# Hiroto1201/Open3D-ML

Measured on AMD Instinct MI355X. Metric: Mpoints/s neighbor-search + sparse-conv fwd; RandLA-Net frames/s, higher is better.
Workload: dtype f32; 1 GPU; C1 fixed_radius_search: layers.FixedRadiusSearch forward (hash build + search) over 64 scenes/GPU x 65,536 U[0,1)^3 pts, r=0.05, L2, int32 idx; scenes_per_gpu=64, parallelism=scene-dp1

## Files before the change

### open3d-ml_amd/csrc/nns_frs.hip

```cpp
#include <algorithm>
#include <cstdlib>
#include <mutex>

#include "primitives.hpp"
#include "spatial_hash.hpp"

namespace o3dml {

__global__ void __launch_bounds__(256) gather_sorted_points_kernel(const float* __restrict__ points,
                                                                   const uint32_t* __restrict__ index, int64_t n,
                                                                   float4* __restrict__ out, int sentinel,
                                                                   int64_t* __restrict__ zero_a, int n_zero_a,
                                                                   int64_t* __restrict__ zero_b) {
    const int64_t per = ceil_div(n, static_cast<int64_t>(gridDim.x));
    const int64_t blk = xcd_block();
    const int64_t e = min(n, (blk + 1) * per);
    constexpr int U = 4;
    for (int64_t j0 = blk * per + threadIdx.x; j0 < e; j0 += U * static_cast<int64_t>(blockDim.x)) {
        uint32_t id[U];
#pragma unroll
        for (int u = 0; u < U; ++u) {
            const int64_t j = j0 + u * static_cast<int64_t>(blockDim.x);
            id[u] = j < e ? index[j] : 0u;
        }
        float x[U], y[U], z[U];
#pragma unroll
        for (int u = 0; u < U; ++u) {
            x[u] = points[3 * static_cast<int64_t>(id[u])];
            y[u] = points[3 * static_cast<int64_t>(id[u]) + 1];
            z[u] = points[3 * static_cast<int64_t>(id[u]) + 2];
        }
#pragma unroll
        for (int u = 0; u < U; ++u) {
            const int64_t j = j0 + u * static_cast<int64_t>(blockDim.x);
            if (j < e) out[j] = make_float4(x[u], y[u], z[u], __uint_as_float(id[u]));
        }
    }
    if (blockIdx.x == 0 && threadIdx.x == 0) {
        if (sentinel) {
            const float inf = __builtin_huge_valf();
            out[n] = make_float4(inf, inf, inf, 0.f);
        }
        for (int j = 0; j < n_zero_a; ++j) zero_a[j] = 0;
        if (zero_b) *zero_b = 0;
    }
}

#ifndef O3DML_FRS_ROWCAP
#define O3DML_FRS_ROWCAP 64
#endif
constexpr int kRowCap = O3DML_FRS_ROWCAP;
static_assert(kRowCap >= 1 && kRowCap <= 64, "the row copy takes one row per wave instruction");
constexpr int kDirWords = 24;

struct LaneSplitTab {
    uint32_t v[65];
    constexpr LaneSplitTab() : v() {
        for (int ng = 0; ng <= 64; ++ng) {
            const uint32_t S = ng == 0 ? 64u : 64u / static_cast<uint32_t>(ng);
            v[ng] = S | (((65536u + S - 1u) / S) << 8);
        }
    }
};
__constant__ constexpr LaneSplitTab kLaneSplitTab{};
#define kLaneSplit kLaneSplitTab.v

#ifndef O3DML_DIAG
#define O3DML_DIAG 0
#endif
#ifndef O3DML_STREAM_U
#define O3DML_STREAM_U 2
#endif
#ifndef O3DML_FRS_DMA
#define O3DML_FRS_DMA 0
#endif
typedef __attribute__((address_space(3))) void* frs_lds_ptr;
#ifndef O3DML_FRS_OOBST
#define O3DML_FRS_OOBST 0
#endif
constexpr int kStreamU = O3DML_STREAM_U;
constexpr int kCandCap = 256;

#ifndef O3DML_FRS_DPPMIN
#define O3DML_FRS_DPPMIN 1
#endif
template <int CTRL>
__device__ __forceinline__ float dpp_f(float v) {
    return __int_as_float(__builtin_amdgcn_update_dpp(0, __float_as_int(v), CTRL, 0xF, 0xF, false));
}
#define O3DML_DPP_STEP(NAME, OP, CTRL)                                                                   \
    __device__ __forceinline__ float NAME(float v) {                                                    \
        float r;                                                                                        \
        asm volatile("s_nop 1\n\t" OP "_dpp %0, %1, %1 " CTRL " row_mask:0xf bank_mask:0xf"            \
                     : "=v"(r)                                                                          \
                     : "v"(v));                                                                         \
        return r;                                                                                       \
    }
O3DML_DPP_STEP(dmin_q1, "v_min_f32", "quad_perm:[1,0,3,2]")
O3DML_DPP_STEP(dmin_q2, "v_min_f32", "quad_perm:[2,3,0,1]")
O3DML_DPP_STEP(dmin_hm, "v_min_f32", "row_half_mirror")
O3DML_DPP_STEP(dmin_rm, "v_min_f32", "row_mirror")
O3DML_DPP_STEP(dmax_q1, "v_max_f32", "quad_perm:[1,0,3,2]")
O3DML_DPP_STEP(dmax_q2, "v_max_f32", "quad_perm:[2,3,0,1]")
O3DML_DPP_STEP(dmax_hm, "v_max_f32", "row_half_mirror")
O3DML_DPP_STEP(dmax_rm, "v_max_f32", "row_mirror")
#undef O3DML_DPP_STEP
template <bool MAX>
__device__ __forceinline__ float row_ext_f(float v) {
#if O3DML_FRS_DPPMIN
    if constexpr (MAX) return dmax_rm(dmax_hm(dmax_q2(dmax_q1(v))));
    return dmin_rm(dmin_hm(dmin_q2(dmin_q1(v))));
#else
    auto op = [](float a, float b) { return MAX ? fmaxf(a, b) : fminf(a, b); };
    v = op(v, dpp_f<0xB1>(v));
    v = op(v, dpp_f<0x4E>(v));
    v = op(v, dpp_f<0x141>(v));
    v = op(v, dpp_f<0x140>(v));
    return v;
#endif
}
__device__ __forceinline__ float rdlane_f(float v, int l) {
    return __int_as_float(__builtin_amdgcn_readlane(__float_as_int(v), l));
}
__device__ __forceinline__ float wave_min_f(float v) {
    v = row_ext_f<false>(v);
    return fminf(fminf(rdlane_f(v, 0), rdlane_f(v, 16)), fminf(rdlane_f(v, 32), rdlane_f(v, 48)));
}
__device__ __forceinline__ float wave_max_f(float v) {
    v = row_ext_f<true>(v);
    return fmaxf(fmaxf(rdlane_f(v, 0), rdlane_f(v, 16)), fmaxf(rdlane_f(v, 32), rdlane_f(v, 48)));
}
__device__ __forceinline__ float row0_min_f(float v) { return rdlane_f(row_ext_f<false>(v), 0); }
__device__ __forceinline__ float row0_max_f(float v) { return rdlane_f(row_ext_f<true>(v), 0); }

template <int METRIC>
__device__ __forceinline__ float box_dist(const float4& p, float lx, float ly, float lz, float hx, float hy,
                                          float hz) {
    const float gx = p.x - __builtin_amdgcn_fmed3f(p.x, lx, hx);
    const float gy = p.y - __builtin_amdgcn_fmed3f(p.y, ly, hy);
    const float gz = p.z - __builtin_amdgcn_fmed3f(p.z, lz, hz);
    if constexpr (METRIC == kL2) {
        return __builtin_fmaf(gz, gz, __builtin_fmaf(gy, gy, gx * gx));
    } else if constexpr (METRIC == kL1) {
        return (fabsf(gx) + fabsf(gy)) + fabsf(gz);
    } else {
        const float ax = fabsf(gx), ay = fabsf(gy), az = fabsf(gz);
        const float m = ax > ay ? ax : ay;
        return m > az ? m : az;
    }
}

template <int METRIC>
__device__ __forceinline__ float box_box_dist(float alx, float aly, float alz, float ahx, float ahy, float ahz,
                                              float blx, float bly, float blz, float bhx, float bhy, float bhz) {
    const float gx = fmaxf(fmaxf(alx - bhx, blx - ahx), 0.f);
    const float gy = fmaxf(fmaxf(aly - bhy, bly - ahy), 0.f);
    const float gz = fmaxf(fmaxf(alz - bhz, blz - ahz), 0.f);
    if constexpr (METRIC == kL2) {
        return __builtin_fmaf(gz, gz, __builtin_fmaf(gy, gy, gx * gx));
    } else if constexpr (METRIC == kL1) {
        return (gx + gy) + gz;
    } else {
        const float m = gx > gy ? gx : gy;
        return m > gz ? m : gz;
    }
}

__device__ __forceinline__ int keep_slot(uint64_t km) {
    return static_cast<int>(__builtin_amdgcn_mbcnt_hi(static_cast<uint32_t>(km >> 32),
                                                      __builtin_amdgcn_mbcnt_lo(static_cast<uint32_t>(km), 0u)));
}

__device__ __forceinline__ uint32_t mbcnt64(uint64_t m) {
    return __builtin_amdgcn_mbcnt_hi(static_cast<uint32_t>(m >> 32),
                                     __builtin_amdgcn_mbcnt_lo(static_cast<uint32_t>(m), 0u));
}

__device__ __forceinline__ uint32_t bcnt_add(uint32_t x, uint32_t acc) {
    uint32_t r;
    asm("v_bcnt_u32_b32 %0, %1, %2" : "=v"(r) : "v"(x), "v"(acc));
    return r;
}

__device__ __forceinline__ uint32_t rdlane(int v, uint32_t lane) {
    return static_cast<uint32_t>(__builtin_amdgcn_readlane(v, static_cast<int>(lane)));
}

__device__ __forceinline__ int32_t float_key(float f) {
    const int32_t i = __float_as_int(f);
    return i ^ ((i >> 31) & 0x7fffffff);
}
__device__ __forceinline__ uint32_t key_float(int32_t k) {
    return static_cast<uint32_t>(k ^ ((k >> 31) & 0x7fffffff));
}

#ifndef O3DML_FRS_NUM_SGPR
#define O3DML_FRS_NUM_SGPR 80
#endif
#ifndef O3DML_FRS_WAVES
#define O3DML_FRS_WAVES 8
#endif
#ifndef O3DML_FRS_ABS16
#define O3DML_FRS_ABS16 1
#endif
#define O3DML_FRS_ATTR \
    __attribute__((amdgpu_num_sgpr(O3DML_FRS_NUM_SGPR), amdgpu_waves_per_eu(DIST ? 1 : O3DML_FRS_WAVES, 8)))
template <int METRIC, bool IGNORE, bool DIST, int MODE, class TIdx, bool REL16>
__global__ void __launch_bounds__(64) O3DML_FRS_ATTR
frs_group_kernel(const float4* __restrict__ pts, uint32_t n_pts, const uint32_t* __restrict__ cs,
                 const float4* __restrict__ qpts, const uint32_t* __restrict__ qsel,
                 const uint32_t* __restrict__ qkeys, int bshift, int64_t m_host, const int64_t* __restrict__ m_dev,
                 float r, float inv, float thr, int nb, const int64_t* __restrict__ qrs,
                 const uint32_t* __restrict__ hts, const int64_t* __restrict__ prs,
                 uint32_t* __restrict__ counts, uint32_t* __restrict__ tidx,
                 float* __restrict__ tdist, uint32_t* __restrict__ over, int64_t* __restrict__ n_over,
                 const int64_t* __restrict__ rs, TIdx* __restrict__ out_idx, float* __restrict__ out_dist,
                 const int64_t* __restrict__ total, int64_t cap, const uint32_t* __restrict__ dir,
                 int64_t dir_cap, int qlog, int64_t dense_w) {
    __shared__ float4 cand[kCandCap];
    __shared__ float4 qsh[64];
    __shared__ int64_t qrow[MODE == 0 ? 1 : 64];
    const int lane = threadIdx.x;
    const float inf = __builtin_huge_valf();
    const float4 far = make_float4(inf, inf, inf, 0.f);
    const int64_t m = MODE == 1 && cap >= 0 && *total > cap ? 0 : (m_dev ? *m_dev : m_host);
    const int64_t nchunks = MODE == 0 ? (m + (1 << qlog) - 1) >> qlog : m;
    const bool pts_rsrc_ok = n_pts < 0x07FFFFFEu;
    const bool sub = dir != nullptr && static_cast<int64_t>(hts[nb]) <= dir_cap;
    const __amdgpu_buffer_rsrc_t rows_rsrc = __builtin_amdgcn_make_buffer_rsrc(
            tidx, static_cast<short>(0), REL16 ? static_cast<int>(m * 2 * kRowCap) : 0, kBufferFlags);
    const __amdgpu_buffer_rsrc_t pts_rsrc = __builtin_amdgcn_make_buffer_rsrc(
            const_cast<float4*>(pts), static_cast<short>(0), static_cast<int>((2u * n_pts + 1u) * 16u), kBufferFlags);
    const int64_t per = (nchunks + 7) >> 3;
    const bool xcd_map = static_cast<int64_t>(gridDim.x) == 8 * per;
    int64_t chunk = xcd_map ? static_cast<int64_t>(blockIdx.x & 7) * per + (blockIdx.x >> 3) : blockIdx.x;
    for (; chunk < nchunks; chunk = xcd_map ? nchunks : chunk + gridDim.x) {
        const int64_t t = MODE == 0 ? (chunk << qlog) + lane : chunk;
        const bool valid = t < m && (MODE == 0 ? lane < (1 << qlog) : lane == 0);
        float4 q4 = far;
        QueryBins qb;
#pragma unroll
        for (int k = 0; k < 9; ++k) qb.b[k] = 0xffffffffu;
        int64_t row = 0;
        uint32_t pbase = 0;
        if (valid) {
            if constexpr (MODE == 0) {
                if (qsel) {
                    const uint32_t qs = qsel[t];
                    if (qpts) {
                        const float* qp = reinterpret_cast<const float*>(qpts) + 3 * static_cast<int64_t>(qs);
                        q4 = make_float4(qp[0], qp[1], qp[2], __uint_as_float(qs));
                    } else {
                        q4 = pts[qs];
                    }
                } else {
                    q4 = qpts[t];
                }
            } else {
                const uint32_t id = over[t];
                const float* qp = reinterpret_cast<const float*>(qpts) + 3 * static_cast<int64_t>(id);
                q4 = make_float4(qp[0], qp[1], qp[2], __uint_as_float(id));
            }
            const uint32_t qid = __float_as_uint(q4.w);
            const int b = qkeys ? (bshift >= 32 ? 0 : static_cast<int>(qkeys[t] >> bshift)) : batch_of(qid, qrs, nb);
            if constexpr (REL16) pbase = static_cast<uint32_t>(prs[b]);
            const uint32_t first = hts[b], tsize = hts[b + 1] - first;
            qb = query_bins(q4.x, q4.y, q4.z, r, inv, first, tsize);
            if constexpr (MODE == 1) row = dense_w > 0 ? static_cast<int64_t>(qid) * dense_w : rs[qid];
        }
        uint64_t todo = __builtin_amdgcn_ballot_w64(valid);
        int ngrp = 0;
        uint32_t goff = 0;
        uint32_t mytag = 0;
        int vgrp = 0;
        while (todo) {
            const int leader = __builtin_ctzll(todo);
            bool same = valid;
#pragma unroll
            for (int k = 0; k < 9; ++k) same = same && qb.b[k] == rdlane(static_cast<int>(qb.b[k]), leader);
            const uint64_t gm = __builtin_amdgcn_ballot_w64(same);
            todo &= ~gm;
            const uint32_t ng = static_cast<uint32_t>(__popcll(gm));
            if (same) {
                const uint32_t slot = mbcnt64(gm);
                mytag = static_cast<uint32_t>(ngrp) | (slot == 0 ? 0x300u : 0x200u) | ((goff + slot) << 16);
            }
            if (lane == ngrp) vgrp = static_cast<int>(ng | (goff << 8) | (static_cast<uint32_t>(leader) << 16));
            goff += ng;
            ++ngrp;
        }
        uint32_t* const tab = reinterpret_cast<uint32_t*>(cand);
        __syncthreads();
        if (valid) {
            qsh[mytag >> 16] = q4;
            if constexpr (MODE == 1) qrow[mytag >> 16] = row;
        }
        uint32_t vst = 0, vlen = 0;
        uint64_t km = 0;
        int gi = 0, nbat = 0;
        for (int grp = 0; grp < ngrp; ++grp, ++gi) {
            if (gi == nbat) {
                uint2* const seg = reinterpret_cast<uint2*>(cand) + 64;
                int bl = lane;
                uint32_t kmax = INT32_MAX, kmin = static_cast<uint32_t>(INT32_MIN), zero = 0u;
                asm volatile("" : "+v"(bl), "+v"(kmax), "+v"(kmin), "+v"(zero));
                const int tg = (bl * 57) >> 9, tk = bl - 9 * tg;
                __syncthreads();
                const uint32_t rel = (mytag & 0xffu) - static_cast<uint32_t>(grp);
                if ((mytag & 0x100u) != 0u && rel < 7u) {
                    uint4* const tp = reinterpret_cast<uint4*>(tab) + 4 * rel;
                    tp[0] = make_uint4(kmax, kmax, kmax, kmin);
                    tp[1] = make_uint4(kmin, kmin, qb.b[0], qb.b[1]);
                    tp[2] = make_uint4(qb.b[2], qb.b[3], qb.b[4], qb.b[5]);
                    tp[3] = make_uint4(qb.b[6], qb.b[7], qb.b[8], zero);
                }
                seg[bl] = make_uint2(zero, zero);
                __syncthreads();
                if ((mytag & 0x200u) != 0u && rel < 7u) {
                    const float4 me = qsh[mytag >> 16];
                    int32_t* const k = reinterpret_cast<int32_t*>(tab) + 16 * rel;
                    const int32_t kx = float_key(me.x), ky = float_key(me.y), kz = float_key(me.z);
                    __hip_atomic_fetch_min(k + 0, kx, __ATOMIC_RELAXED, __HIP_MEMORY_SCOPE_WORKGROUP);
                    __hip_atomic_fetch_min(k + 1, ky, __ATOMIC_RELAXED, __HIP_MEMORY_SCOPE_WORKGROUP);
                    __hip_atomic_fetch_min(k + 2, kz, __ATOMIC_RELAXED, __HIP_MEMORY_SCOPE_WORKGROUP);
                    __hip_atomic_fetch_max(k + 3, kx, __ATOMIC_RELAXED, __HIP_MEMORY_SCOPE_WORKGROUP);
                    __hip_atomic_fetch_max(k + 4, ky, __ATOMIC_RELAXED, __HIP_MEMORY_SCOPE_WORKGROUP);
                    __hip_atomic_fetch_max(k + 5, kz, __ATOMIC_RELAXED, __HIP_MEMORY_SCOPE_WORKGROUP);
                }
                __syncthreads();
                const bool task_ok = tg < 7 && grp + tg < ngrp;
                const uint32_t* const tq = tab + 16 * tg;
                const uint32_t vb = tab[task_ok ? 16 * tg + 6 + tk : 6];
                const uint32_t prev = tq[5 + tk];
                const uint4 b0 = reinterpret_cast<const uint4*>(tq)[0];
                const uint2 b1 = reinterpret_cast<const uint2*>(tq)[2];
                const uint32_t s0 = cs[vb], e0 = cs[vb + 1];
                uint4 w0 = {}, w1 = {}, w2 = {}, w3 = {}, w4 = {}, w5 = {};
                if (sub) {
                    const uint4* dp = reinterpret_cast<const uint4*>(dir + static_cast<size_t>(vb) * kDirWords);
                    w0 = dp[0], w1 = dp[1], w2 = dp[2], w3 = dp[3], w4 = dp[4], w5 = dp[5];
                }
                const bool first = task_ok && e0 > s0 && (tk == 0 || prev != vb);
                uint32_t st = s0, ln = e0 - s0;
                if (first && sub) {
                    auto f = [](uint32_t u) { return __uint_as_float(u); };
                    auto kf = [](uint32_t k) { return __uint_as_float(key_float(static_cast<int32_t>(k))); };
                    const float lx = kf(b0.x), ly = kf(b0.y), lz = kf(b0.z), hx = kf(b0.w), hy = kf(b1.x),
                                hz = kf(b1.y);
                    const uint32_t n0 = w0.x, n1 = w0.y, n2 = ln - n0 - n1;
                    const bool r0 = n0 > 0 && box_box_dist<METRIC>(f(w1.x), f(w1.y), f(w1.z), f(w1.w), f(w2.x),
                                                                   f(w2.y), lx, ly, lz, hx, hy, hz) <= thr;
                    const bool r1 = n1 > 0 && box_box_dist<METRIC>(f(w2.z), f(w2.w), f(w3.x), f(w3.y), f(w3.z),
                                                                   f(w3.w), lx, ly, lz, hx, hy, hz) <= thr;
                    const bool r2 = n2 > 0 && box_box_dist<METRIC>(f(w4.x), f(w4.y), f(w4.z), f(w4.w), f(w5.x),
                                                                   f(w5.y), lx, ly, lz, hx, hy, hz) <= thr;
                    const int nr = static_cast<int>(r0) + static_cast<int>(r1) + static_cast<int>(r2);
                    const uint32_t base = n_pts + 1 + s0;
                    if (nr == 0) {
                        ln = 0;
                    } else if (nr == 1) {
                        st = r0 && n0 == ln ? s0 : base + (r0 ? 0u : (r1 ? n0 : n0 + n1));
                        ln = r0 ? n0 : (r1 ? n1 : n2);
                    }
                }
                const bool live = first && ln > 0;
                km = __builtin_amdgcn_ballot_w64(live);
                nbat = __popcll(km) > 57 ? 6 : min(7, ngrp - grp);
                if (live && tg < nbat) seg[mbcnt64(km) + tg] = make_uint2(st, ln);
                __syncthreads();
                const uint2 sg = seg[bl];
                vst = sg.x, vlen = sg.y;
                __syncthreads();
                gi = 0;
            }
            const uint32_t ginfo = rdlane(vgrp, static_cast<uint32_t>(grp));
            const int ng = static_cast<int>(ginfo & 0xffu);
            const uint32_t gslot = (ginfo >> 8) & 0xffu, leader = ginfo >> 16;
            const uint32_t gbase = REL16 ? rdlane(static_cast<int>(pbase), leader) : 0u;
            float lx, ly, lz, hx, hy, hz;
            if (ng <= 16) {
                const float4 v = lane < ng ? qsh[gslot + (lane & 15)] : far;
                const float4 w = lane < ng ? v : make_float4(-inf, -inf, -inf, 0.f);
                lx = row0_min_f(v.x), ly = row0_min_f(v.y), lz = row0_min_f(v.z);
                hx = row0_max_f(w.x), hy = row0_max_f(w.y), hz = row0_max_f(w.z);
            } else {
                const float4 v = lane < ng ? qsh[gslot + lane] : far;
                const float4 w = lane < ng ? v : make_float4(-inf, -inf, -inf, 0.f);
                lx = wave_min_f(v.x), ly = wave_min_f(v.y), lz = wave_min_f(v.z);
                hx = wave_max_f(w.x), hy = wave_max_f(w.y), hz = wave_max_f(w.z);
            }
            const uint32_t split = kLaneSplit[ng];
            const int S = static_cast<int>(split & 0xffu);
            const int g = static_cast<int>((static_cast<uint32_t>(lane) * (split >> 8)) >> 16);
            const int sl = lane - g * S;
            float4 mq = far;
            int64_t mrow = 0;
            if (g < ng) {
                mq = qsh[gslot + g];
                mrow = MODE == 0 ? static_cast<int64_t>(__float_as_uint(mq.w)) : qrow[gslot + g];
            }
            uint32_t cnt = 0;
            const uint32_t row_b = static_cast<uint32_t>(mrow) * (2u * kRowCap);
            const uint64_t gmask = S == 64 ? ~0ull : (g < ng ? ((1ull << S) - 1ull) << (g * S) : 0ull);
            const uint32_t gm_lo = static_cast<uint32_t>(gmask), gm_hi = static_cast<uint32_t>(gmask >> 32);
            int bk = __popcll(km & ((1ull << (9 * gi)) - 1ull)) + gi;
            int nbk = bk + __popcll((km >> (9 * gi)) & 0x1ffull);
#if O3DML_DIAG == 2
            nbk = bk;
#endif
            const int fill_lim = kCandCap - 64 * kStreamU - (S - 1);
            uint32_t boff = 0;
            auto round_src = [&]() -> uint32_t {
                if (bk >= nbk) return n_pts;
                const uint32_t st0 = rdlane(static_cast<int>(vst), bk) + boff;
                const uint32_t t = rdlane(static_cast<int>(vlen), bk) - boff;
                if (t > 64) {
                    boff += 64;
                    return st0 + lane;
                }
                const uint32_t n1 = rdlane(static_cast<int>(vlen), bk + 1);
                const uint32_t d1 = rdlane(static_cast<int>(vst), bk + 1) - t;
                const uint32_t src = static_cast<uint32_t>(lane) < t ? st0 + lane : d1 + lane;
                if (t + n1 <= 64) {
                    bk += 2;
                    boff = 0;
                } else {
                    bk += 1;
                    boff = 64 - t;
                }
                return static_cast<uint32_t>(lane) < t + n1 ? src : n_pts;
            };
            auto load_step = [&](float4* c, auto buf) {
                uint32_t src[kStreamU];
#pragma unroll
                for (int u = 0; u < kStreamU; ++u) src[u] = round_src();
                if constexpr (decltype(buf)::value) {
#pragma unroll
                    for (int u = 0; u < kStreamU; ++u)
                        c[u] = __builtin_bit_cast(float4,
                                                  __builtin_amdgcn_raw_buffer_load_b128(pts_rsrc, src[u] * 16u, 0, 0));
                } else {
#pragma unroll
                    for (int u = 0; u < kStreamU; ++u) c[u] = pts[src[u]];
                }
            };
            auto stream_and_test = [&](auto buf) {
            int nc = 0;
            while (true) {
#if O3DML_FRS_DMA
                if constexpr (decltype(buf)::value) {
                    while (bk < nbk && nc <= fill_lim) {
                        uint32_t src[kStreamU];
#pragma unroll
                        for (int u = 0; u < kStreamU; ++u) src[u] = round_src();
                        const int nc0 = nc;
#pragma unroll
                        for (int u = 0; u < kStreamU; ++u)
                            __builtin_amdgcn_raw_ptr_buffer_load_lds(pts_rsrc, (frs_lds_ptr)(cand + nc0 + 64 * u), 16,
                                                                     src[u] * 16u, 0, 0, 0);
                        asm volatile("s_waitcnt vmcnt(0)" ::: "memory");
#pragma unroll
                        for (int u = 0; u < kStreamU; ++u) {
                            float4 c = cand[nc0 + 64 * u + lane];
                            const bool keep = box_dist<METRIC>(c, lx, ly, lz, hx, hy, hz) <= thr;
                            const uint64_t km = __builtin_amdgcn_ballot_w64(keep);
                            if constexpr (REL16 && !O3DML_FRS_ABS16) c.w = __uint_as_float(__float_as_uint(c.w) - gbase);
                            if (keep)
                                (cand + nc)[keep_slot(km)] = c;
                            nc += __popcll(km);
                        }
                    }
                }
                while (!decltype(buf)::value && bk < nbk && nc <= fill_lim) {
#else
                while (bk < nbk && nc <= fill_lim) {
#endif
                    float4 c[kStreamU];
                    load_step(c, buf);
#pragma unroll
                    for (int u = 0; u < kStreamU; ++u) {
                        const bool keep = box_dist<METRIC>(c[u], lx, ly, lz, hx, hy, hz) <= thr;
                        const uint64_t km = __builtin_amdgcn_ballot_w64(keep);
                        if constexpr (REL16 && !O3DML_FRS_ABS16)
                            c[u].w = __uint_as_float(__float_as_uint(c[u].w) - gbase);
                        if (keep)
                            (cand + nc)[keep_slot(km)] = c[u];
                        nc += __popcll(km);
                    }
                }
                const int ncp = static_cast<int>(((static_cast<uint32_t>(nc + S - 1) * (split >> 8)) >> 16) *
                                                 static_cast<uint32_t>(S));
                if (nc + lane < ncp) cand[nc + lane] = far;
                __syncthreads();
#if O3DML_DIAG == 0
                auto test = [&](float4 p) {
                    asm volatile("" : "+v"(p.w));
                    const float d = dist_metric<METRIC>(p.x, p.y, p.z, mq.x, mq.y, mq.z);
                    const bool hit = d <= thr && !(IGNORE && p.x == mq.x && p.y == mq.y && p.z == mq.z);
                    const uint64_t bal = __builtin_amdgcn_ballot_w64(hit);
                    const uint32_t mlo = static_cast<uint32_t>(bal) & gm_lo;
                    const uint32_t mhi = static_cast<uint32_t>(bal >> 32) & gm_hi;
#if O3DML_FRS_OOBST
                    if constexpr (MODE == 0 && REL16 && !DIST) {
                        const uint32_t pos = __builtin_amdgcn_mbcnt_hi(mhi, __builtin_amdgcn_mbcnt_lo(mlo, cnt));
                        const uint32_t ps = min(pos, static_cast<uint32_t>(kRowCap - 1));
                        __builtin_amdgcn_raw_buffer_store_b16(static_cast<unsigned short>(__float_as_uint(p.w)),
                                                              rows_rsrc, hit ? row_b + (ps << 1) : 0x80000000u, 0,
                                                              0);
                        cnt = bcnt_add(mhi, bcnt_add(mlo, cnt));
                        return;
                    }
#endif
                    if (hit) {
                        const uint32_t pos = __builtin_amdgcn_mbcnt_hi(mhi, __builtin_amdgcn_mbcnt_lo(mlo, cnt));
                        if constexpr (MODE == 0) {
                            const uint32_t ps = min(pos, static_cast<uint32_t>(kRowCap - 1));
                            if constexpr (REL16)
                                __builtin_amdgcn_raw_buffer_store_b16(
                                        static_cast<unsigned short>(__float_as_uint(p.w)), rows_rsrc,
                                        row_b + (ps << 1), 0, 0);
                            else
                                tidx[mrow * kRowCap + ps] = __float_as_uint(p.w);
                            if constexpr (DIST) tdist[mrow * kRowCap + ps] = d;
                        } else {
                            out_idx[mrow + pos] = static_cast<TIdx>(__float_as_uint(p.w));
                            if constexpr (DIST) out_dist[mrow + pos] = d;
                        }
                    }
                    cnt = bcnt_add(mhi, bcnt_add(mlo, cnt));
                };
                int e0 = 0;
                for (; e0 + 4 * S <= ncp; e0 += 4 * S) {
                    float4 p[4];
#pragma unroll
                    for (int u = 0; u < 4; ++u) p[u] = cand[e0 + u * S + sl];
#pragma unroll
                    for (int u = 0; u < 4; ++u) test(p[u]);
                }
                for (; e0 < ncp; e0 += S) test(cand[e0 + sl]);
#endif
                __syncthreads();
                nc = 0;
                if (bk >= nbk) break;
            }
            };
            if (pts_rsrc_ok)
                stream_and_test(std::true_type{});
            else
                stream_and_test(std::false_type{});
            if constexpr (MODE == 0) {
                if (g < ng && sl == 0) {
                    counts[__float_as_uint(mq.w)] = cnt;
                    if (cnt > static_cast<uint32_t>(kRowCap))
                        over[atomicAdd(reinterpret_cast<unsigned long long*>(n_over), 1ull)] =
                                static_cast<uint32_t>(mrow);
                }
            }
        }
    }
}

__device__ uint32_t g_frs_zero[4];
#ifndef O3DML_COPY_ROWS
#define O3DML_COPY_ROWS 64
#endif
constexpr int kCopyRows = O3DML_COPY_ROWS;

template <bool DIST, bool REL16, class TIdx>
__global__ void __launch_bounds__(256) group_rows_copy_kernel(int64_t m, const uint32_t* __restrict__ counts,
                                                              const int64_t* __restrict__ rs,
                                                              const int64_t* __restrict__ qrs,
                                                              const int64_t* __restrict__ prs, int nb,
                                                              const uint32_t* __restrict__ tidx,
                                                              const float* __restrict__ tdist,
                                                              TIdx* __restrict__ idx, float* __restrict__ dist,
                                                              int64_t cap) {
    if (cap >= 0 && rs[m] > cap) return;
    const int lane = threadIdx.x & 63;
    const int64_t wave = (static_cast<int64_t>(blockIdx.x) * blockDim.x + threadIdx.x) >> 6;
    const int64_t nwaves = (static_cast<int64_t>(gridDim.x) * blockDim.x) >> 6;
    const uint16_t* t16 = reinterpret_cast<const uint16_t*>(tidx);
    for (int64_t base = wave * 64; base < m; base += nwaves * 64) {
        const int64_t t = base + lane;
        int n = 0;
        int64_t o = 0;
        uint32_t pb = 0;
        if constexpr (REL16) {
            const int64_t ub = static_cast<int64_t>(__builtin_amdgcn_readfirstlane(static_cast<int>(base >> 6))) << 6;
            const int b0 = batch_of(ub, qrs, nb);
            const int64_t last = min(ub + 63, m - 1);
            pb = static_cast<uint32_t>(prs[b0]);
            if (qrs[b0 + 1] <= last && t < m) pb = static_cast<uint32_t>(prs[batch_of(t, qrs, nb)]);
        }
        if (t < m) {
            const uint32_t c = counts[t];
            n = c <= static_cast<uint32_t>(kRowCap) ? static_cast<int>(c) : 0;
            o = rs[t];
        }
        for (int k = 0; k < 64; k += kCopyRows) {
            uint32_t v[kCopyRows];
            float dv[kCopyRows];
#pragma unroll
            for (int u = 0; u < kCopyRows; ++u) {
                const int nu = __builtin_amdgcn_readlane(n, k + u);
                const int64_t src = (base + k + u) * kRowCap + lane;
                const bool live = lane < nu;
                if constexpr (REL16)
                    v[u] = *(live ? t16 + src : reinterpret_cast<const uint16_t*>(g_frs_zero));
                else
                    v[u] = *(live ? tidx + src : g_frs_zero);
                if constexpr (DIST) dv[u] = *(live ? tdist + src : reinterpret_cast<const float*>(g_frs_zero));
            }
#pragma unroll
            for (int u = 0; u < kCopyRows; ++u) {
                const int nu = __builtin_amdgcn_readlane(n, k + u);
                const int64_t ou = static_cast<int64_t>(
                        (static_cast<uint64_t>(static_cast<uint32_t>(__builtin_amdgcn_readlane(static_cast<int>(o >> 32), k + u))) << 32) |
                        static_cast<uint32_t>(__builtin_amdgcn_readlane(static_cast<int>(o), k + u)));
                const uint32_t pbu = REL16 ? static_cast<uint32_t>(__builtin_amdgcn_readlane(static_cast<int>(pb), k + u)) : 0u;
                if (lane < nu) {
                    idx[ou + lane] = static_cast<TIdx>(O3DML_FRS_ABS16 && REL16 ? pbu + ((v[u] - pbu) & 0xffffu)
                                                                                 : v[u] + pbu);
                    if constexpr (DIST) dist[ou + lane] = dv[u];
                }
            }
        }
    }
}

template <bool REL16>
__global__ void __launch_bounds__(256) group_rows_dense_kernel(int64_t m, const uint32_t* __restrict__ counts,
                                                               const int64_t* __restrict__ qrs,
                                                               const int64_t* __restrict__ prs, int nb,
                                                               const uint32_t* __restrict__ tidx, int64_t width,
                                                               int32_t pad, int32_t* __restrict__ out) {
    const int lane = threadIdx.x & 63;
    const int64_t nwaves = (static_cast<int64_t>(gridDim.x) * blockDim.x) >> 6;
    const uint16_t* t16 = reinterpret_cast<const uint16_t*>(tidx);
    for (int64_t t = (static_cast<int64_t>(blockIdx.x) * blockDim.x + threadIdx.x) >> 6; t < m; t += nwaves) {
        const uint32_t c = counts[t];
        const int64_t n = c <= static_cast<uint32_t>(kRowCap) ? static_cast<int64_t>(c) : 0;
        const int64_t n_all = static_cast<int64_t>(c);
        const uint32_t pb = REL16 ? static_cast<uint32_t>(prs[batch_of(t, qrs, nb)]) : 0u;
        int32_t* row = out + t * width;
        for (int64_t j = lane; j < width; j += 64) {
            if (j < n)
                row[j] = static_cast<int32_t>(REL16 ? (O3DML_FRS_ABS16 ? pb + ((t16[t * kRowCap + j] - pb) & 0xffffu)
                                                                       : t16[t * kRowCap + j] + pb)
                                                    : tidx[t * kRowCap + j]);
            else if (j >= n_all)
                row[j] = pad;
        }
    }
}

__device__ __forceinline__ uint32_t spread3(uint32_t v) {
    v &= 0x3ffu;
    v = (v | (v << 16)) & 0x030000FFu;
    v = (v | (v << 8)) & 0x0300F00Fu;
    v = (v | (v << 4)) & 0x030C30C3u;
    v = (v | (v << 2)) & 0x09249249u;
    return v;
}

template <bool F4>
__global__ void __launch_bounds__(256) group_query_keys_kernel(const float* __restrict__ queries, int64_t m,
                                                               float inv2, int n_batch,
                                                               const int64_t* __restrict__ qrs, int cell_bits,
                                                               uint32_t* __restrict__ keys) {
    __shared__ int64_t s_rs[kLdsSplits];
    const int64_t* rsp = stage_splits(s_rs, qrs, n_batch);
    const uint32_t mask = (1u << cell_bits) - 1u;
    constexpr int W = F4 ? 4 : 3;
    for (int64_t i = blockIdx.x * static_cast<int64_t>(blockDim.x) + threadIdx.x; i < m;
         i += static_cast<int64_t>(gridDim.x) * blockDim.x) {
        const int b = batch_of(i, rsp, n_batch);
        float x, y, z;
        if constexpr (F4) {
            const float4 p = reinterpret_cast<const float4*>(queries)[i];
            x = p.x, y = p.y, z = p.z;
        } else {
            x = queries[W * i], y = queries[W * i + 1], z = queries[W * i + 2];
        }
        const uint32_t cx = static_cast<uint32_t>(static_cast<int32_t>(floorf(x * inv2))) & mask;
        const uint32_t cy = static_cast<uint32_t>(static_cast<int32_t>(floorf(y * inv2))) & mask;
        const uint32_t cz = static_cast<uint32_t>(static_cast<int32_t>(floorf(z * inv2))) & mask;
        const uint32_t mort = spread3(cx) | (spread3(cy) << 1) | (spread3(cz) << 2);
        keys[i] = (static_cast<uint32_t>(b) << (3 * cell_bits)) | mort;
    }
}

constexpr int kSelfChunk = 256;

template <bool MAX>
// ... 766 lines not shown
```

Baseline: 4149 Mpoints/s.

## Group queries by run detection and reuse batch bounding boxes from LDS

Replaces the serial per-leader ballot loop that groups lanes sharing the same 9 hash bins with a one-shot run detection. It compares each lane with its left neighbour via DPP and uses a hashed LDS table to confirm that runs are unique, falling back to the old loop otherwise. The per-group query bounding box, previously rebuilt with DPP min/max reductions, is now read from the batch key box already staged in LDS and broadcast with readlane. The lane-split lookup is also hoisted out of the group loop. This adds extra syncthreads and LDS traffic, and the box used for pruning may be looser (cell-level rather than a tight query box), which could add more candidate work.

```diff
diff --git a/open3d-ml_amd/csrc/nns_frs.hip b/open3d-ml_amd/csrc/nns_frs.hip
--- a/open3d-ml_amd/csrc/nns_frs.hip
+++ b/open3d-ml_amd/csrc/nns_frs.hip
@@ -80,58 +80,15 @@
 #endif
 constexpr int kStreamU = O3DML_STREAM_U;
 constexpr int kCandCap = 256;
-
-#ifndef O3DML_FRS_DPPMIN
-#define O3DML_FRS_DPPMIN 1
-#endif
-template <int CTRL>
-__device__ __forceinline__ float dpp_f(float v) {
-    return __int_as_float(__builtin_amdgcn_update_dpp(0, __float_as_int(v), CTRL, 0xF, 0xF, false));
-}
-#define O3DML_DPP_STEP(NAME, OP, CTRL)                                                                   \
-    __device__ __forceinline__ float NAME(float v) {                                                    \
-        float r;                                                                                        \
-        asm volatile("s_nop 1\n\t" OP "_dpp %0, %1, %1 " CTRL " row_mask:0xf bank_mask:0xf"            \
-                     : "=v"(r)                                                                          \
-                     : "v"(v));                                                                         \
-        return r;                                                                                       \
-    }
-O3DML_DPP_STEP(dmin_q1, "v_min_f32", "quad_perm:[1,0,3,2]")
-O3DML_DPP_STEP(dmin_q2, "v_min_f32", "quad_perm:[2,3,0,1]")
-O3DML_DPP_STEP(dmin_hm, "v_min_f32", "row_half_mirror")
-O3DML_DPP_STEP(dmin_rm, "v_min_f32", "row_mirror")
-O3DML_DPP_STEP(dmax_q1, "v_max_f32", "quad_perm:[1,0,3,2]")
-O3DML_DPP_STEP(dmax_q2, "v_max_f32", "quad_perm:[2,3,0,1]")
-O3DML_DPP_STEP(dmax_hm, "v_max_f32", "row_half_mirror")
-O3DML_DPP_STEP(dmax_rm, "v_max_f32", "row_mirror")
-#undef O3DML_DPP_STEP
-template <bool MAX>
-__device__ __forceinline__ float row_ext_f(float v) {
-#if O3DML_FRS_DPPMIN
-    if constexpr (MAX) return dmax_rm(dmax_hm(dmax_q2(dmax_q1(v))));
-    return dmin_rm(dmin_hm(dmin_q2(dmin_q1(v))));
-#else
-    auto op = [](float a, float b) { return MAX ? fmaxf(a, b) : fminf(a, b); };
-    v = op(v, dpp_f<0xB1>(v));
-    v = op(v, dpp_f<0x4E>(v));
-    v = op(v, dpp_f<0x141>(v));
-    v = op(v, dpp_f<0x140>(v));
-    return v;
-#endif
+constexpr uint32_t kRunSlot0 = 512, kRunSlots = 512;
+
+__device__ __forceinline__ uint32_t left_lane(uint32_t v) {
+    return static_cast<uint32_t>(
+            __builtin_amdgcn_update_dpp(static_cast<int>(v), static_cast<int>(v), 0x138, 0xF, 0xF, false));
 }
 __device__ __forceinline__ float rdlane_f(float v, int l) {
     return __int_as_float(__builtin_amdgcn_readlane(__float_as_int(v), l));
 }
-__device__ __forceinline__ float wave_min_f(float v) {
-    v = row_ext_f<false>(v);
-    return fminf(fminf(rdlane_f(v, 0), rdlane_f(v, 16)), fminf(rdlane_f(v, 32), rdlane_f(v, 48)));
-}
-__device__ __forceinline__ float wave_max_f(float v) {
-    v = row_ext_f<true>(v);
-    return fmaxf(fmaxf(rdlane_f(v, 0), rdlane_f(v, 16)), fmaxf(rdlane_f(v, 32), rdlane_f(v, 48)));
-}
-__device__ __forceinline__ float row0_min_f(float v) { return rdlane_f(row_ext_f<false>(v), 0); }
-__device__ __forceinline__ float row0_max_f(float v) { return rdlane_f(row_ext_f<true>(v), 0); }
 
 template <int METRIC>
 __device__ __forceinline__ float box_dist(const float4& p, float lx, float ly, float lz, float hx, float hy,
@@ -268,34 +225,60 @@
             qb = query_bins(q4.x, q4.y, q4.z, r, inv, first, tsize);
             if constexpr (MODE == 1) row = dense_w > 0 ? static_cast<int64_t>(qid) * dense_w : rs[qid];
         }
-        uint64_t todo = __builtin_amdgcn_ballot_w64(valid);
-        int ngrp = 0;
-        uint32_t goff = 0;
-        uint32_t mytag = 0;
-        int vgrp = 0;
-        while (todo) {
-            const int leader = __builtin_ctzll(todo);
-            bool same = valid;
-#pragma unroll
-            for (int k = 0; k < 9; ++k) same = same && qb.b[k] == rdlane(static_cast<int>(qb.b[k]), leader);
-            const uint64_t gm = __builtin_amdgcn_ballot_w64(same);
-            todo &= ~gm;
-            const uint32_t ng = static_cast<uint32_t>(__popcll(gm));
-            if (same) {
-                const uint32_t slot = mbcnt64(gm);
-                mytag = static_cast<uint32_t>(ngrp) | (slot == 0 ? 0x300u : 0x200u) | ((goff + slot) << 16);
-            }
-            if (lane == ngrp) vgrp = static_cast<int>(ng | (goff << 8) | (static_cast<uint32_t>(leader) << 16));
-            goff += ng;
-            ++ngrp;
-        }
+        bool lead = lane == 0;
+#pragma unroll
+        for (int k = 0; k < 9; ++k) lead |= qb.b[k] != left_lane(qb.b[k]);
+        lead &= valid;
+        const uint64_t lm = __builtin_amdgcn_ballot_w64(lead);
+        uint32_t hs = qb.b[0];
+#pragma unroll
+        for (int k = 1; k < 9; ++k) hs += qb.b[k] << k;
+        hs = kRunSlot0 + ((hs ^ (hs >> 9)) & (kRunSlots - 1u));
+        int ngrp = __popcll(lm);
+        uint32_t mytag = valid ? mbcnt64(lm) + (lead ? 0x300u : 0x1ffu) + (static_cast<uint32_t>(lane) << 16) : 0u;
         uint32_t* const tab = reinterpret_cast<uint32_t*>(cand);
         __syncthreads();
+        if (lead) {
+            tab[mytag & 0xffu] = static_cast<uint32_t>(lane);
+            tab[hs] = static_cast<uint32_t>(lane);
+        }
+        __syncthreads();
+        int vgrp = 0;
+        if (__builtin_amdgcn_ballot_w64(lead && tab[hs] != static_cast<uint32_t>(lane)) == 0) {
+            const uint32_t nvalid = static_cast<uint32_t>(__popcll(__builtin_amdgcn_ballot_w64(valid)));
+            if (lane < ngrp) {
+                const uint32_t l0 = tab[lane];
+                const uint32_t l1 = lane + 1 < ngrp ? tab[lane + 1] : nvalid;
+                vgrp = static_cast<int>((l1 - l0) | (l0 << 8) | (l0 << 16));
+            }
+        } else {
+            uint64_t todo = __builtin_amdgcn_ballot_w64(valid);
+            uint32_t goff = 0;
+            ngrp = 0;
+            while (todo) {
+                const int leader = __builtin_ctzll(todo);
+                bool same = valid;
+#pragma unroll
+                for (int k = 0; k < 9; ++k) same = same && qb.b[k] == rdlane(static_cast<int>(qb.b[k]), leader);
+                const uint64_t gm = __builtin_amdgcn_ballot_w64(same);
+                todo &= ~gm;
+                const uint32_t ng = static_cast<uint32_t>(__popcll(gm));
+                if (same) {
+                    const uint32_t slot = mbcnt64(gm);
+                    mytag = static_cast<uint32_t>(ngrp) | (slot == 0 ? 0x300u : 0x200u) | ((goff + slot) << 16);
+                }
+                if (lane == ngrp) vgrp = static_cast<int>(ng | (goff << 8) | (static_cast<uint32_t>(leader) << 16));
+                goff += ng;
+                ++ngrp;
+            }
+        }
+        const int vsplit = static_cast<int>(kLaneSplit[vgrp & 0xff]);
         if (valid) {
             qsh[mytag >> 16] = q4;
             if constexpr (MODE == 1) qrow[mytag >> 16] = row;
         }
         uint32_t vst = 0, vlen = 0;
+        float vbox = 0.f;
         uint64_t km = 0;
         int gi = 0, nbat = 0;
         for (int grp = 0; grp < ngrp; ++grp, ++gi) {
@@ -334,6 +317,7 @@
                 const uint32_t prev = tq[5 + tk];
                 const uint4 b0 = reinterpret_cast<const uint4*>(tq)[0];
                 const uint2 b1 = reinterpret_cast<const uint2*>(tq)[2];
+                vbox = __uint_as_float(key_float(static_cast<int32_t>(tab[16 * (bl >> 3) + (bl & 7)])));
                 const uint32_t s0 = cs[vb], e0 = cs[vb + 1];
                 uint4 w0 = {}, w1 = {}, w2 = {}, w3 = {}, w4 = {}, w5 = {};
                 if (sub) {
@@ -377,19 +361,12 @@
             const int ng = static_cast<int>(ginfo & 0xffu);
             const uint32_t gslot = (ginfo >> 8) & 0xffu, leader = ginfo >> 16;
             const uint32_t gbase = REL16 ? rdlane(static_cast<int>(pbase), leader) : 0u;
-            float lx, ly, lz, hx, hy, hz;
-            if (ng <= 16) {
-                const float4 v = lane < ng ? qsh[gslot + (lane & 15)] : far;
-                const float4 w = lane < ng ? v : make_float4(-inf, -inf, -inf, 0.f);
-                lx = row0_min_f(v.x), ly = row0_min_f(v.y), lz = row0_min_f(v.z);
-                hx = row0_max_f(w.x), hy = row0_max_f(w.y), hz = row0_max_f(w.z);
-            } else {
-                const float4 v = lane < ng ? qsh[gslot + lane] : far;
-                const float4 w = lane < ng ? v : make_float4(-inf, -inf, -inf, 0.f);
-                lx = wave_min_f(v.x), ly = wave_min_f(v.y), lz = wave_min_f(v.z);
-                hx = wave_max_f(w.x), hy = wave_max_f(w.y), hz = wave_max_f(w.z);
-            }
-            const uint32_t split = kLaneSplit[ng];
+            const float lx = rdlane_f(vbox, 8 * gi), ly = rdlane_f(vbox, 8 * gi + 1),
+                        lz = rdlane_f(vbox, 8 * gi + 2);
+            float hx = rdlane_f(vbox, 8 * gi + 3), hy = rdlane_f(vbox, 8 * gi + 4),
+                  hz = rdlane_f(vbox, 8 * gi + 5);
+            asm volatile("" : "+v"(hx), "+v"(hy), "+v"(hz));
+            const uint32_t split = rdlane(vsplit, static_cast<uint32_t>(grp));
             const int S = static_cast<int>(split & 0xffu);
             const int g = static_cast<int>((static_cast<uint32_t>(lane) * (split >> 8)) >> 16);
             const int sl = lane - g * S;
```

Measured after the change: 4204 Mpoints/s, median of 6. +1.3%, better.
